# NJU-3DV/Relightable3DGaussian

Hardware: AMD Instinct MI355X
Metric: train iters/s, synthetic lego-like 800x800, 300000 Gaussians (stage-2 hot path) (higher is better)
Workload: dtype f32; 1 GPU; stage-2 train iteration (fused glue kernels + one-launch Adam): shading fwd/bwd (K=64) + rasterize fwd (S=16) + loss + rasterize bwd + Adam; 1 view/rank/step, 300000 Gaussians, 800x800, num_rendered~1755022; parallelism=dp1

## Files before the change

include/r3dg_hip.h:

```cpp
#ifndef R3DG_HIP_H
#define R3DG_HIP_H

#include <stddef.h>
#include <stdint.h>

#ifdef __cplusplus
extern "C" {
#endif

#define R3DG_OK 0
#define R3DG_EINVAL (-1)
#define R3DG_EHIP (-2)
#define R3DG_EALLOC (-3)

typedef void* (*r3dg_alloc_fn)(void* user, size_t bytes);

const char* r3dg_last_error(void);
int r3dg_release_scratch(void);
int r3dg_version(void);

int r3dg_max_features_forward(void);
int r3dg_max_features_backward(void);

size_t r3dg_geometry_state_bytes(int P);
// ... 24 lines not shown
                                 const float* d_rotations, const float* d_cov3D_precomp, const float* d_viewmatrix,
                                 const float* d_projmatrix, const float* d_cam_pos, float tan_fovx, float tan_fovy,
                                 float cx, float cy, int prefiltered, int compute_pseudo_normal, float* d_out_color,
                                 float* d_out_opacity, float* d_out_depth, float* d_out_feature, float* d_out_normal,
                                 float* d_out_surface_xyz, float* d_out_weights, int32_t* d_radii, int debug,
                                 void** ticket);
int r3dg_rasterize_forward_finish(void* ticket, int* num_rendered_out);
int r3dg_rasterize_forward_finish_on(void* ticket, void* ordering_stream, int* num_rendered_out);

int r3dg_bounded_forward_supported(int width, int height);
int r3dg_rasterize_forward_begin_bounded(void* stream, r3dg_alloc_fn geometry_alloc, r3dg_alloc_fn binning_alloc,
                                         r3dg_alloc_fn image_alloc, void* alloc_user, int P, int S, int D, int M,
                                         const float* d_background, int width, int height, const float* d_means3D,
                                         const float* d_shs, const float* d_colors_precomp, const float* d_features,
                                         const float* d_opacities, const float* d_scales, float scale_modifier,
                                         const float* d_rotations, const float* d_cov3D_precomp,
                                         const float* d_viewmatrix, const float* d_projmatrix, const float* d_cam_pos,
                                         float tan_fovx, float tan_fovy, float cx, float cy, int prefiltered,
                                         int compute_pseudo_normal, float* d_out_color, float* d_out_opacity,
                                         float* d_out_depth, float* d_out_feature, float* d_out_normal,
                                         float* d_out_surface_xyz, float* d_out_weights, int32_t* d_radii, int debug,
                                         void* ordering_stream, long long capacity, float* d_overflow_flag,
                                         unsigned int* d_overflow_count, void** ticket);
int r3dg_rasterize_forward_finish_bounded(void* ticket, void* main_stream);

int r3dg_rasterize_backward(void* stream, int P, int S, int D, int M, int R, const float* d_background, int width,
                            int height, const float* d_means3D, const float* d_shs, const float* d_features,
                            const float* d_colors_precomp, const float* d_scales, float scale_modifier,
                            const float* d_rotations, const float* d_cov3D_precomp, const float* d_viewmatrix,
                            const float* d_projmatrix, const float* d_campos, float tan_fovx, float tan_fovy,
                            const int32_t* d_radii, const void* d_geom_buffer, const void* d_binning_buffer,
                            const void* d_img_buffer, const float* d_dL_dpix, const float* d_dL_dpix_o,
                            const float* d_dL_dpix_d, const float* d_dL_dpix_f, float* d_dL_dmean2D,
                            float* d_dL_dconic, float* d_dL_dopacity, float* d_dL_dcolor, float* d_dL_dfeature,
                            float* d_dL_dmean3D, float* d_dL_dcov3D, float* d_dL_dsh, float* d_dL_dscale,
                            float* d_dL_drot, int backward_geometry, int debug);

int r3dg_rasterize_backward_split(void* stream, void* geometry_stream, int P, int S, int D, int M, int R,
                                  const float* d_background, int width, int height, const float* d_means3D,
                                  const float* d_shs, const float* d_features, const float* d_colors_precomp,
                                  const float* d_scales, float scale_modifier, const float* d_rotations,
                                  const float* d_cov3D_precomp, const float* d_viewmatrix, const float* d_projmatrix,
                                  const float* d_campos, float tan_fovx, float tan_fovy, const int32_t* d_radii,
                                  const void* d_geom_buffer, const void* d_binning_buffer, const void* d_img_buffer,
                                  const float* d_dL_dpix, const float* d_dL_dpix_o, const float* d_dL_dpix_d,
                                  const float* d_dL_dpix_f, float* d_dL_dmean2D, float* d_dL_dconic,
// ... 328 lines not shown
```

relightable3dgaussian_amd/csrc/capi_rasterizer.hip:

```cpp
#include "capi_internal.hpp"

#include <mutex>
#include <vector>

namespace r3dg {

GeometryLayout GeometryLayout::make(size_t P)
{
    GeometryLayout L;
    size_t o = 0;
    auto take = [&](size_t bytes) { size_t r = o; o = align_up(o + bytes, 256); return r; };
    L.depths = take(P * 4);
    L.clamped = take(P * 3);
    L.radii = take(P * 4);
    L.means2D = take(P * 8);
    L.cov3D = take(P * 24);
    L.conic_opacity = take(P * 16);
    L.rgb = take(P * 12);
    L.tiles_touched = take(P * 4);
    L.point_offsets = take(P * 4);
    L.block_sums = take(((P + 255) / 256 + 1) * 4);
    L.total = take(8);
    L.splat = take(P * 64);
    L.bytes = o;
// ... 51 lines not shown
        return RasterView{gx, gy, T, N, GeometryLayout::make((size_t)P), ImageLayout::make(N, T)};
    }
};

struct ForwardArgs {
    void* stream;
    r3dg_alloc_fn geometry_alloc, binning_alloc, image_alloc;
    void* user;
    int P, S, D, M;
    const float* background;
    int width, height;
    const float *means3D, *shs, *colors_precomp, *features, *opacities, *scales;
    float scale_modifier;
    const float *rotations, *cov3D_precomp, *viewmatrix, *projmatrix, *cam_pos;
    float tan_fovx, tan_fovy, cx, cy;
    int prefiltered, compute_pseudo_normal;
    float *out_color, *out_opacity, *out_depth, *out_feature, *out_normal, *out_surface_xyz, *out_weights;
    int32_t* radii;
    int debug;
    long long capacity;
    float* overflow_flag;
    unsigned int* overflow_count;
    void* ordering_stream;
};

struct ForwardTicket {
    ForwardArgs a;
    RasterView v;
    float focal_x, focal_y;
    int* radii_p;
    char *gbuf, *ibuf;
    hipEvent_t ready, ordered;
    unsigned long long* host_total;
    char* bbuf;
    bool fused_front;
    uint32_t* point_list;
};

static std::mutex g_ticket_mutex;
static std::vector<ForwardTicket*> g_ticket_pool;

static ForwardTicket* ticket_acquire()
{
    {
        std::lock_guard<std::mutex> lk(g_ticket_mutex);
        if (!g_ticket_pool.empty()) {
// ... 138 lines not shown

    return guarded([&]() -> int {
        hipStream_t stream = (hipStream_t)a.stream;
        const bool debug = a.debug != 0;
        const RasterView v = RasterView::make(a.P, a.width, a.height);
        const GeometryLayout& G = v.G;
        char* gbuf = (char*)a.geometry_alloc(a.user, G.bytes);
        char* ibuf = (char*)a.image_alloc(a.user, v.I.bytes);
        if (!gbuf || !ibuf) { set_error("rasterize_forward: resize callback returned NULL"); return R3DG_EALLOC; }

        ForwardTicket* t = ticket_acquire();
        struct Release { ForwardTicket* t; ~Release() { if (t) ticket_release(t); } } on_error{t};
        t->a = a;
        t->v = v;
        t->focal_y = a.height / (2.0f * a.tan_fovy);
        t->focal_x = a.width / (2.0f * a.tan_fovx);
        t->radii_p = a.radii ? a.radii : (int*)(gbuf + G.radii);
        t->gbuf = gbuf;
        t->ibuf = ibuf;
        t->bbuf = nullptr;
        t->fused_front = false;
        t->point_list = nullptr;
        const hipStream_t order_stream = a.capacity >= 0 && a.ordering_stream ? (hipStream_t)a.ordering_stream : stream;
        stream_wait_stream(order_stream, stream);
        uint32_t* zero_words = nullptr;
        int zero_n = 0;
        if (a.capacity >= 0 && direct_binning_usable((long long)v.T)) {
            BinningLayout B = BinningLayout::make((size_t)a.capacity);
            t->bbuf = (char*)a.binning_alloc(a.user, B.bytes);
            if (!t->bbuf) { set_error("rasterize_forward: binning resize callback returned NULL"); return R3DG_EALLOC; }
            t->fused_front = true;
            zero_words = (uint32_t*)(t->bbuf + B.sort_temp);
            zero_n = (int)v.T;
        }
        unsigned long long* g_total = (unsigned long long*)(gbuf + G.total);
        StageTimer t_pre(order_stream, ST_PREPROCESS);
        launch_preprocess(order_stream, a.P, a.D, a.M, a.means3D, a.scales, a.scale_modifier, a.rotations, a.opacities, a.shs,
                          (uint8_t*)(gbuf + G.clamped), a.cov3D_precomp, a.colors_precomp, a.viewmatrix, a.projmatrix,
                          a.cam_pos, a.width, a.height, a.tan_fovx, a.tan_fovy, t->focal_x, t->focal_y, t->radii_p,
                          (float*)(gbuf + G.means2D), (float*)(gbuf + G.depths), (float*)(gbuf + G.cov3D),
                          (float*)(gbuf + G.rgb), (float*)(gbuf + G.conic_opacity), (float*)(gbuf + G.splat), v.gx, v.gy,
                          (uint32_t*)(gbuf + G.tiles_touched), (uint32_t*)(gbuf + G.block_sums), g_total, !t->fused_front,
                          zero_words, zero_n);
        check_launch(order_stream, debug, "preprocess");
        t_pre.stop();

        if (a.capacity >= 0) {
            const int st_order = enqueue_ordering(t, order_stream, (int)a.capacity);
            if (st_order != R3DG_OK) return st_order;
            R3DG_HIP(hipEventRecord(t->ordered, order_stream));
        } else {
            R3DG_HIP(hipMemcpyAsync(t->host_total, g_total, sizeof(unsigned long long), hipMemcpyDeviceToHost, stream));
            R3DG_HIP(hipEventRecord(t->ready, stream));
        }
        on_error.t = nullptr;
        *ticket_out = t;
        return R3DG_OK;
    });
}

}

using namespace r3dg;

extern "C" {

// ... 34 lines not shown
{
    BinningLayout L = BinningLayout::make((size_t)R);
    o[0] = L.keys_unsorted; o[1] = L.keys; o[2] = L.vals_unsorted; o[3] = L.vals;
    return R3DG_OK;
}

#define R3DG_FORWARD_ARGS                                                                                              \
    stream_, geometry_alloc, binning_alloc, image_alloc, user, P, S, D, M, background, width, height, means3D, shs,    \
        colors_precomp, features, opacities, scales, scale_modifier, rotations, cov3D_precomp, viewmatrix, projmatrix, \
        cam_pos, tan_fovx, tan_fovy, cx, cy, prefiltered, compute_pseudo_normal, out_color, out_opacity, out_depth,    \
        out_feature, out_normal, out_surface_xyz, out_weights, radii, debug_

int r3dg_rasterize_forward_begin(void* stream_, r3dg_alloc_fn geometry_alloc, r3dg_alloc_fn binning_alloc,
                           r3dg_alloc_fn image_alloc, void* user, int P, int S, int D, int M,
                           const float* background, int width, int height, const float* means3D, const float* shs,
                           const float* colors_precomp, const float* features, const float* opacities,
                           const float* scales, float scale_modifier, const float* rotations,
                           const float* cov3D_precomp, const float* viewmatrix, const float* projmatrix,
                           const float* cam_pos, float tan_fovx, float tan_fovy, float cx, float cy, int prefiltered,
                           int compute_pseudo_normal, float* out_color, float* out_opacity, float* out_depth,
                           float* out_feature, float* out_normal, float* out_surface_xyz, float* out_weights,
                           int32_t* radii, int debug_, void** ticket_out)
{
    return forward_begin_impl(ForwardArgs{R3DG_FORWARD_ARGS, -1, nullptr, nullptr, nullptr}, ticket_out);
}

int r3dg_rasterize_forward_begin_bounded(void* stream_, r3dg_alloc_fn geometry_alloc, r3dg_alloc_fn binning_alloc,
                           r3dg_alloc_fn image_alloc, void* user, int P, int S, int D, int M,
                           const float* background, int width, int height, const float* means3D, const float* shs,
                           const float* colors_precomp, const float* features, const float* opacities,
                           const float* scales, float scale_modifier, const float* rotations,
                           const float* cov3D_precomp, const float* viewmatrix, const float* projmatrix,
                           const float* cam_pos, float tan_fovx, float tan_fovy, float cx, float cy, int prefiltered,
                           int compute_pseudo_normal, float* out_color, float* out_opacity, float* out_depth,
                           float* out_feature, float* out_normal, float* out_surface_xyz, float* out_weights,
                           int32_t* radii, int debug_, void* ordering_stream, long long capacity,
                           float* overflow_flag, unsigned int* overflow_count, void** ticket_out)
{
    if (capacity < 0 || capacity > 0x7fffffffll) return invalid("rasterize_forward (bounded): capacity must be in [0, 2^31)");
    return forward_begin_impl(ForwardArgs{R3DG_FORWARD_ARGS, capacity, overflow_flag, overflow_count, ordering_stream},
                              ticket_out);
}
int r3dg_rasterize_forward_finish_bounded(void* ticket_, void* main_stream_)
{
    if (!ticket_) return R3DG_OK;
    ForwardTicket* t = (ForwardTicket*)ticket_;
    if (t->a.capacity < 0) return invalid("rasterize_forward_finish_bounded: not a bounded ticket");
    const int st = guarded([&]() -> int {
        const hipStream_t stream = (hipStream_t)main_stream_;
        R3DG_HIP(hipStreamWaitEvent(stream, t->ordered, 0));
        render_tiles(t, stream);
        return R3DG_OK;
    });
    ticket_release(t);
    return st;
}

int r3dg_rasterize_forward_finish(void* ticket_, int* num_rendered_out)
{
    return r3dg_rasterize_forward_finish_on(ticket_, nullptr, num_rendered_out);
}

int r3dg_rasterize_forward_finish_on(void* ticket_, void* ordering_stream_, int* num_rendered_out)
// ... 16 lines not shown
        if (st_order != R3DG_OK) return st_order;
        stream_wait_stream(main_stream, order_stream);
        render_tiles(t, main_stream);
        if (num_rendered_out) *num_rendered_out = R;
        return R3DG_OK;
    });
    ticket_release(t);
    return st;
}

int r3dg_rasterize_forward(void* stream_, r3dg_alloc_fn geometry_alloc, r3dg_alloc_fn binning_alloc,
                           r3dg_alloc_fn image_alloc, void* user, int P, int S, int D, int M,
                           const float* background, int width, int height, const float* means3D, const float* shs,
                           const float* colors_precomp, const float* features, const float* opacities,
                           const float* scales, float scale_modifier, const float* rotations,
                           const float* cov3D_precomp, const float* viewmatrix, const float* projmatrix,
                           const float* cam_pos, float tan_fovx, float tan_fovy, float cx, float cy, int prefiltered,
                           int compute_pseudo_normal, float* out_color, float* out_opacity, float* out_depth,
                           float* out_feature, float* out_normal, float* out_surface_xyz, float* out_weights,
                           int32_t* radii, int debug_, int* num_rendered_out)
{
    if (num_rendered_out) *num_rendered_out = 0;
    void* ticket = nullptr;
    const int st = forward_begin_impl(ForwardArgs{R3DG_FORWARD_ARGS, -1, nullptr, nullptr, nullptr}, &ticket);
    if (st != R3DG_OK) return st;
    return r3dg_rasterize_forward_finish(ticket, num_rendered_out);
}
#undef R3DG_FORWARD_ARGS

int r3dg_rasterize_backward(void* stream_, int P, int S, int D, int M, int R, const float* background, int width,
                            int height, const float* means3D, const float* shs, const float* features,
                            const float* colors_precomp, const float* scales, float scale_modifier,
                            const float* rotations, const float* cov3D_precomp, const float* viewmatrix,
                            const float* projmatrix, const float* campos, float tan_fovx, float tan_fovy,
                            const int32_t* radii, const void* geom_buffer, const void* binning_buffer,
                            const void* img_buffer, const float* dL_dpix, const float* dL_dpix_o,
                            const float* dL_dpix_d, const float* dL_dpix_f, float* dL_dmean2D, float* dL_dconic,
                            float* dL_dopacity, float* dL_dcolor, float* dL_dfeature, float* dL_dmean3D,
                            float* dL_dcov3D, float* dL_dsh, float* dL_dscale, float* dL_drot,
                            int backward_geometry, int debug_)
{
    return r3dg_rasterize_backward_split(stream_, stream_, P, S, D, M, R, background, width, height, means3D, shs,
                                         features, colors_precomp, scales, scale_modifier, rotations, cov3D_precomp,
                                         viewmatrix, projmatrix, campos, tan_fovx, tan_fovy, radii, geom_buffer,
                                         binning_buffer, img_buffer, dL_dpix, dL_dpix_o, dL_dpix_d, dL_dpix_f, dL_dmean2D,
                                         dL_dconic, dL_dopacity, dL_dcolor, dL_dfeature, dL_dmean3D, dL_dcov3D, dL_dsh,
                                         dL_dscale, dL_drot, backward_geometry, debug_, -1, nullptr);
// ... 138 lines not shown
```

relightable3dgaussian_amd/csrc/launchers.hpp:

```cpp
#pragma once
#include "common.hpp"

namespace r3dg {

constexpr int REFILL_MIN_IDLE = 16;

void release_gradient_records();
void launch_mark_visible(hipStream_t s, int P, const float* means3D, const float* vm, uint8_t* present);
void launch_preprocess(hipStream_t s, int P, int D, int M, const float* means3D, const float* scales, float scale_modifier,
                       const float* rotations, const float* opacities, const float* shs, uint8_t* clamped,
                       const float* cov3D_precomp, const float* colors_precomp, const float* vm, const float* pm,
                       const float* cam_pos, int W, int H, float tan_fovx, float tan_fovy, float focal_x, float focal_y,
                       int* radii, float* means2D, float* depths, float* cov3Ds, float* rgb, float* conic_opacity,
                       float* splat, int gx, int gy, uint32_t* tiles_touched, uint32_t* block_sums,
                       unsigned long long* total, bool scan_now, uint32_t* zero_words, int zero_n);
void launch_duplicate_with_keys(hipStream_t s, int P, const float* means2D, const float* depths,
                                const uint32_t* tiles_touched, const uint32_t* block_offsets, uint32_t* point_offsets,
                                uint64_t* keys, uint32_t* values, const int* radii, int gx, int gy);
void launch_identify_tile_ranges(hipStream_t s, int L, const uint64_t* keys, uint32_t* ranges);
void launch_tile_order(hipStream_t s, int T, const uint32_t* ranges, uint32_t* order, uint32_t small_cap, uint32_t* big_list,
                       uint32_t* big_count);
void launch_render_forward(hipStream_t s, int W, int H, int S, const uint32_t* tile_order, const uint32_t* ranges,
                           const uint32_t* point_list, const float* splat, const float* features, float* final_T,
                           uint32_t* n_contrib, const float* bg, float* out_color, float* out_opacity, float* out_depth,
                           float* out_feature, float* out_weights);
void launch_pseudo_normal(hipStream_t s, int W, int H, const float* vm, float focal_x, float focal_y, float cx, float cy,
                          const float* opacities, const float* depths, float* normals, float* surface_xyz, bool debug);
void launch_render_backward(hipStream_t s, int P, int W, int H, int S, int n_active, const int* active,
                            const uint32_t* tile_order, const uint32_t* ranges, const uint32_t* point_list, const float* bg,
                            const float* splat, const float* features, const float* final_Ts, const uint32_t* n_contrib,
                            const float* dL_dpix, const float* dL_dpix_o, const float* dL_dpix_d, const float* dL_dpix_f,
                            float* dL_dmean2D, float* dL_dconic, float* dL_dopacity, float* dL_dcolor, float* dL_dfeature,
                            int bg_geom);
void launch_render_backward_features(hipStream_t s, int W, int H, int S, int n_active, const int* active,
                                     const uint32_t* tile_order, const uint32_t* ranges, const uint32_t* point_list,
                                     const float* splat, const float* final_Ts, const uint32_t* n_contrib,
                                     const float* dL_dpix_f, float* dL_dfeature);
void launch_preprocess_backward(hipStream_t s, int P, int D, int M, const float* means, const int* radii, const float* shs,
// ... 185 lines not shown
```

relightable3dgaussian_amd/csrc/rasterizer_preprocess.hip:

```cpp
#include <atomic>

#include "launchers.hpp"

namespace r3dg {

struct M3 {
    float c[3][3];
};
__device__ __forceinline__ M3 m3mul(const M3& A, const M3& B)
{
    M3 R;
#pragma unroll
    for (int j = 0; j < 3; j++)
#pragma unroll
        for (int i = 0; i < 3; i++)
            R.c[j][i] = A.c[0][i] * B.c[j][0] + A.c[1][i] * B.c[j][1] + A.c[2][i] * B.c[j][2];
    return R;
}
__device__ __forceinline__ M3 m3t(const M3& A)
{
    M3 R;
#pragma unroll
    for (int j = 0; j < 3; j++)
#pragma unroll
// ... 18 lines not shown
    y0 = min(gy, max(0, f2i_sat((py - max_radius) / R3DG_TILE_Y)));
    x1 = min(gx, max(0, f2i_sat((px + max_radius + R3DG_TILE_X - 1) / R3DG_TILE_X)));
    y1 = min(gy, max(0, f2i_sat((py + max_radius + R3DG_TILE_Y - 1) / R3DG_TILE_Y)));
}

__constant__ float kSH_C0 = 0.28209479177387814f;
__constant__ float kSH_C1 = 0.4886025119029199f;
__constant__ float kSH_C2[5] = {1.0925484305920792f, -1.0925484305920792f, 0.31539156525252005f,
                                -1.0925484305920792f, 0.5462742152960396f};
__constant__ float kSH_C3[7] = {-0.5900435899266435f, 2.890611442640554f, -0.4570457994644658f,
                                0.3731763325901154f, -0.4570457994644658f, 1.445305721320277f,
                                -0.5900435899266435f};

__global__ void mark_visible_kernel(int P, const float* __restrict__ pts, const float* __restrict__ vm,
                                    uint8_t* __restrict__ present)
{
    int idx = blockIdx.x * blockDim.x + threadIdx.x;
    if (idx >= P) return;
    float x = pts[3 * idx], y = pts[3 * idx + 1], z = pts[3 * idx + 2];
    float vz = vm[2] * x + vm[6] * y + vm[10] * z + vm[14];
    present[idx] = vz > 0.2f;
}

template <bool STAGED>
__global__ void __launch_bounds__(256)
preprocess_kernel(int P, int D, int M, const float* __restrict__ means3D, const float* __restrict__ scales,
                  float scale_modifier, const float* __restrict__ rotations, const float* __restrict__ opacities,
                  const float* __restrict__ shs, uint8_t* __restrict__ clamped, const float* __restrict__ cov3D_precomp,
                  const float* __restrict__ colors_precomp, const float* __restrict__ vm,
                  const float* __restrict__ pm, const float* __restrict__ cam_pos, int W, int H, float tan_fovx,
                  float tan_fovy, float focal_x, float focal_y, int* __restrict__ radii,
                  float2* __restrict__ means2D, float* __restrict__ depths, float* __restrict__ cov3Ds,
                  float* __restrict__ rgb, float4* __restrict__ conic_opacity, float4* __restrict__ splat, int gx, int gy,
                  uint32_t* __restrict__ tiles_touched, uint32_t* __restrict__ block_sums,
                  uint32_t* __restrict__ zero_words, int zero_n)
{
    extern __shared__ float s_rows[];
    __shared__ uint8_t s_live[256];
    const int idx = blockIdx.x * 256 + threadIdx.x;
    if (idx < zero_n) zero_words[idx] = 0u;
    uint32_t my_tiles = 0;
    bool shade = false;
    float px = 0.f, py = 0.f, pz = 0.f;
    float4 rec0 = make_float4(0.f, 0.f, 0.f, 0.f), rec1 = rec0;
    if (idx < P) {
        int my_radius_i = 0;
        do {
            px = means3D[3 * idx]; py = means3D[3 * idx + 1]; pz = means3D[3 * idx + 2];
            const float vx = vm[0] * px + vm[4] * py + vm[8] * pz + vm[12];
            const float vy = vm[1] * px + vm[5] * py + vm[9] * pz + vm[13];
            const float vz = vm[2] * px + vm[6] * py + vm[10] * pz + vm[14];
            if (vz <= 0.2f) break;
            const float hx = pm[0] * px + pm[4] * py + pm[8] * pz + pm[12];
            const float hy = pm[1] * px + pm[5] * py + pm[9] * pz + pm[13];
            const float hw = pm[3] * px + pm[7] * py + pm[11] * pz + pm[15];
            const float p_w = 1.0f / (hw + 0.0000001f);
            const float projx = hx * p_w, projy = hy * p_w;

            float c3[6];
            if (cov3D_precomp != nullptr) {
#pragma unroll
                for (int i = 0; i < 6; i++) c3[i] = cov3D_precomp[6 * idx + i];
            } else {
                const float sx = scale_modifier * scales[3 * idx], sy = scale_modifier * scales[3 * idx + 1],
                            sz = scale_modifier * scales[3 * idx + 2];
                const float r = rotations[4 * idx], x = rotations[4 * idx + 1], y = rotations[4 * idx + 2],
                            z = rotations[4 * idx + 3];
                M3 S = {{{sx, 0, 0}, {0, sy, 0}, {0, 0, sz}}};
                M3 R = {{{1.f - 2.f * (y * y + z * z), 2.f * (x * y - r * z), 2.f * (x * z + r * y)},
                         {2.f * (x * y + r * z), 1.f - 2.f * (x * x + z * z), 2.f * (y * z - r * x)},
                         {2.f * (x * z - r * y), 2.f * (y * z + r * x), 1.f - 2.f * (x * x + y * y)}}};
                M3 Mm = m3mul(S, R);
                M3 Sg = m3mul(m3t(Mm), Mm);
                c3[0] = Sg.c[0][0]; c3[1] = Sg.c[0][1]; c3[2] = Sg.c[0][2];
                c3[3] = Sg.c[1][1]; c3[4] = Sg.c[1][2]; c3[5] = Sg.c[2][2];
#pragma unroll
                for (int i = 0; i < 6; i++) cov3Ds[6 * idx + i] = c3[i];
            }

            float tx = vx, ty = vy;
            const float tz = vz;
            const float limx = 1.3f * tan_fovx, limy = 1.3f * tan_fovy;
            const float txtz = tx / tz, tytz = ty / tz;
            tx = fminf(limx, fmaxf(-limx, txtz)) * tz;
            ty = fminf(limy, fmaxf(-limy, tytz)) * tz;
            M3 J = {{{focal_x / tz, 0.0f, -(focal_x * tx) / (tz * tz)},
                     {0.0f, focal_y / tz, -(focal_y * ty) / (tz * tz)},
                     {0, 0, 0}}};
            M3 Wm = {{{vm[0], vm[4], vm[8]}, {vm[1], vm[5], vm[9]}, {vm[2], vm[6], vm[10]}}};
            M3 T = m3mul(Wm, J);
            M3 V = {{{c3[0], c3[1], c3[2]}, {c3[1], c3[3], c3[4]}, {c3[2], c3[4], c3[5]}}};
            M3 cov = m3mul(m3mul(m3t(T), m3t(V)), T);
            const float ca = cov.c[0][0] + 0.3f, cb = cov.c[0][1], cc = cov.c[1][1] + 0.3f;

            const float det = (ca * cc - cb * cb);
            if (det == 0.0f) break;
            const float det_inv = 1.f / det;
            const float mid = 0.5f * (ca + cc);
            const float lambda1 = mid + sqrtf(fmaxf(0.1f, mid * mid - det));
            const float lambda2 = mid - sqrtf(fmaxf(0.1f, mid * mid - det));
            const float my_radius = ceilf(3.f * sqrtf(fmaxf(lambda1, lambda2)));
            const float pixx = ndc_to_pix(projx, W), pixy = ndc_to_pix(projy, H);
            int x0, y0, x1, y1;
            tile_rect(pixx, pixy, f2i_sat(my_radius), gx, gy, x0, y0, x1, y1);
            if ((x1 - x0) * (y1 - y0) == 0) break;

            shade = colors_precomp == nullptr;
            depths[idx] = vz;
            my_radius_i = f2i_sat(my_radius);
            means2D[idx] = make_float2(pixx, pixy);
            const float4 co = make_float4(cc * det_inv, -cb * det_inv, ca * det_inv, opacities[idx]);
            conic_opacity[idx] = co;
            rec0 = make_float4(pixx, pixy, co.x, co.y);
            rec1 = make_float4(co.z, co.w, vz, 0.f);
            my_tiles = (uint32_t)((y1 - y0) * (x1 - x0));
        } while (0);
        radii[idx] = my_radius_i;
        tiles_touched[idx] = my_tiles;
    }
    if (STAGED) {
        s_live[threadIdx.x] = shade;
        __syncthreads();
        stage_rows_in_256(shs, blockIdx.x * 256, P, 3 * M, s_live, s_rows);
        __syncthreads();
    }
    float col[3] = {0.f, 0.f, 0.f};
    if (shade) {
        float dx = px - cam_pos[0], dy = py - cam_pos[1], dz = pz - cam_pos[2];
        const float len = sqrtf(dx * dx + dy * dy + dz * dz);
        dx = dx / len; dy = dy / len; dz = dz / len;
        const float* sh = STAGED ? s_rows + threadIdx.x * staged_row_stride(3 * M) : shs + (size_t)idx * M * 3;
#pragma unroll
        for (int ch = 0; ch < 3; ch++) {
            float result = kSH_C0 * sh[ch];
// ... 507 lines not shown
        total, capacity, nb, (const uint2*)ranges, order, small_cap, big_list, big_count);
}

int tile_binning_max_tiles() { return BIN_MAX_TILES; }

void launch_tile_order(hipStream_t s, int T, const uint32_t* ranges, uint32_t* order, uint32_t small_cap,
                       uint32_t* big_list, uint32_t* big_count)
{
    tile_order_kernel<<<1, 1024, 0, s>>>(T, (const uint2*)ranges, order, small_cap, big_list, big_count);
}

void launch_mark_visible(hipStream_t s, int P, const float* means3D, const float* vm, uint8_t* present)
{
    if (P <= 0) return;
    mark_visible_kernel<<<(P + 255) / 256, 256, 0, s>>>(P, means3D, vm, present);
}

void launch_preprocess(hipStream_t s, int P, int D, int M, const float* means3D, const float* scales,
                       float scale_modifier, const float* rotations, const float* opacities, const float* shs,
                       uint8_t* clamped, const float* cov3D_precomp, const float* colors_precomp, const float* vm,
                       const float* pm, const float* cam_pos, int W, int H, float tan_fovx, float tan_fovy,
                       float focal_x, float focal_y, int* radii, float* means2D, float* depths, float* cov3Ds,
                       float* rgb, float* conic_opacity, float* splat, int gx, int gy, uint32_t* tiles_touched,
                       uint32_t* block_sums, unsigned long long* total, bool scan_now, uint32_t* zero_words, int zero_n)
{
    const int nb = (P + 255) / 256;
    if (zero_n > nb * 256) {
        R3DG_HIP(hipMemsetAsync(zero_words, 0, (size_t)zero_n * 4, s));
        zero_n = 0;
    }
    const bool staged = opt(R3DG_OPT_STAGE_SH_ROWS) && shs != nullptr && colors_precomp == nullptr && M >= 1 && M <= 16;
    if (staged)
        preprocess_kernel<true><<<nb, 256, 256 * ((3 * M) | 1) * sizeof(float), s>>>(
            P, D, M, means3D, scales, scale_modifier, rotations, opacities, shs, clamped, cov3D_precomp, colors_precomp,
            vm, pm, cam_pos, W, H, tan_fovx, tan_fovy, focal_x, focal_y, radii, (float2*)means2D, depths, cov3Ds, rgb,
            (float4*)conic_opacity, (float4*)splat, gx, gy, tiles_touched, block_sums, zero_words, zero_n);
    else
        preprocess_kernel<false><<<nb, 256, 0, s>>>(
            P, D, M, means3D, scales, scale_modifier, rotations, opacities, shs, clamped, cov3D_precomp, colors_precomp,
            vm, pm, cam_pos, W, H, tan_fovx, tan_fovy, focal_x, focal_y, radii, (float2*)means2D, depths, cov3Ds, rgb,
            (float4*)conic_opacity, (float4*)splat, gx, gy, tiles_touched, block_sums, zero_words, zero_n);
    if (scan_now) scan_block_sums_kernel<<<1, 1024, 0, s>>>(nb, block_sums, total);
}

void launch_duplicate_with_keys(hipStream_t s, int P, const float* means2D, const float* depths,
                                const uint32_t* tiles_touched, const uint32_t* block_offsets,
                                uint32_t* point_offsets, uint64_t* keys, uint32_t* values, const int* radii, int gx,
                                int gy)
{
    duplicate_with_keys_kernel<<<(P + 255) / 256, 256, 0, s>>>(P, (const float2*)means2D, depths, tiles_touched,
                                                             block_offsets, point_offsets, keys, values, radii, gx, gy);
}

void launch_identify_tile_ranges(hipStream_t s, int L, const uint64_t* keys, uint32_t* ranges)
{
    if (L <= 0) return;
    identify_tile_ranges_kernel<<<(L + 255) / 256, 256, 0, s>>>(L, keys, (uint2*)ranges);
}

}
```

relightable3dgaussian_amd/csrc/stage2_glue.hip:

```cpp
#include <type_traits>

#include "launchers.hpp"
#include "pseudo_normal.hpp"
#include "r3dg_hip.h"

namespace r3dg {

__device__ __forceinline__ float srgb_pow(float x, float y) { return __builtin_amdgcn_exp2f(y * __builtin_amdgcn_logf(x)); }


__device__ __forceinline__ float sigmoidf_(float x) { return 1.f / (1.f + __expf(-x)); }

__device__ __forceinline__ void normalize3(const float v[3], float eps, float out[3], float& inv)
{
    const float n = sqrtf(v[0] * v[0] + v[1] * v[1] + v[2] * v[2]);
    inv = 1.f / fmaxf(n, eps);
    out[0] = v[0] * inv; out[1] = v[1] * inv; out[2] = v[2] * inv;
}
__device__ __forceinline__ void normalize3_backward(const float v[3], float eps, const float g[3], float out[3])
{
    const float n = sqrtf(v[0] * v[0] + v[1] * v[1] + v[2] * v[2]);
    if (n > eps) {
        const float inv = 1.f / n;
        const float u[3] = {v[0] * inv, v[1] * inv, v[2] * inv};
// ... 20 lines not shown
s2_activate_kernel(int P, const float* __restrict__ xyz, const float* __restrict__ scaling_raw,
                   const float* __restrict__ rotation_raw, const float* __restrict__ opacity_raw,
                   const float* __restrict__ normal_raw, const float* __restrict__ base_raw,
                   const float* __restrict__ rough_raw, const float* __restrict__ campos,
                   float* __restrict__ scales, float* __restrict__ rot, float* __restrict__ opacity,
                   float* __restrict__ normal, float* __restrict__ base_color, float* __restrict__ roughness,
                   float* __restrict__ viewdirs, const float* __restrict__ viewmatrix, float* __restrict__ features,
                   ActivateSide side)
{
    if ((int)blockIdx.x >= side.nb_main) {
        const int nb_side = (int)gridDim.x - side.nb_main;
        for (int k = ((int)blockIdx.x - side.nb_main) * 256 + (int)threadIdx.x; k < side.n_env; k += nb_side * 256) {
            const float r = side.env_raw[k];
            side.env[k] = r > 20.f ? r : log1pf(expf(r));
        }
        for (int k = ((int)blockIdx.x - side.nb_main) * 256 + (int)threadIdx.x; k < side.n_zero; k += nb_side * 256)
            side.zero[k] = 0.f;
        return;
    }
    const int i = blockIdx.x * 256 + threadIdx.x;
    if (i >= P) return;
    const size_t i3 = 3 * (size_t)i, i4 = 4 * (size_t)i;
#pragma unroll
    for (int c = 0; c < 3; c++) scales[i3 + c] = __expf(scaling_raw[i3 + c]);
    {
        const float q[4] = {rotation_raw[i4], rotation_raw[i4 + 1], rotation_raw[i4 + 2], rotation_raw[i4 + 3]};
        const float inv = 1.f / fmaxf(sqrtf(q[0] * q[0] + q[1] * q[1] + q[2] * q[2] + q[3] * q[3]), 1e-12f);
#pragma unroll
        for (int c = 0; c < 4; c++) rot[i4 + c] = q[c] * inv;
    }
    opacity[i] = sigmoidf_(opacity_raw[i]);
    float inv, nrm[3];
    {
        const float v[3] = {normal_raw[i3], normal_raw[i3 + 1], normal_raw[i3 + 2]};
        normalize3(v, 1e-3f, nrm, inv);
        normal[i3] = nrm[0]; normal[i3 + 1] = nrm[1]; normal[i3 + 2] = nrm[2];
    }
    if (base_raw != nullptr) {
        float bc[3];
#pragma unroll
        for (int c = 0; c < 3; c++) base_color[i3 + c] = bc[c] = 0.03f + 0.77f * sigmoidf_(base_raw[i3 + c]);
        const float rg = 0.09f + 0.9f * sigmoidf_(rough_raw[i]);
        roughness[i] = rg;
        const float p[3] = {xyz[i3], xyz[i3 + 1], xyz[i3 + 2]};
        const float d[3] = {campos[0] - p[0], campos[1] - p[1], campos[2] - p[2]};
        float o[3];
        normalize3(d, 1e-12f, o, inv);
        viewdirs[i3] = o[0]; viewdirs[i3 + 1] = o[1]; viewdirs[i3 + 2] = o[2];
        if (features != nullptr) {
            const float depth = p[0] * viewmatrix[2] + p[1] * viewmatrix[6] + p[2] * viewmatrix[10] + viewmatrix[14];
            float* f = features + 16 * (size_t)i;
            *reinterpret_cast<float2*>(f) = make_float2(depth, depth * depth);
            f[5] = nrm[0]; f[6] = nrm[1]; f[7] = nrm[2];
            *reinterpret_cast<float4*>(f + 8) = make_float4(bc[0], bc[1], bc[2], rg);
// ... 1296 lines not shown
```

relightable3dgaussian_amd/fused_step.py:

```python
import collections
import contextlib
import os

import torch
import torch.nn.functional as F

from . import _lib, rasterizer_ops, shading_ops
from .fused_adam import AdamGroup, FusedAdam
from .fused_base import _STREAMS, SUM_SLOTS, FusedStepBase, _in_context, _world_of, grad_slab, learning_rates, shared_stream
from .fused_stage1 import FusedStage1Step
from .grad_comm import BucketComm
from .shading_ops import LEAVE_ROOM, TRAIN_OUTPUTS
from .train_step import FROZEN_GEOMETRY_GROUPS, LAMBDA_DSSIM, STAGE2_WEIGHTS, update_visibility

PARAM_NAMES = ("xyz", "normal", "scaling", "rotation", "opacity", "shs", "base_color", "roughness", "incidents", "env")

_View = collections.namedtuple("_View", "cam bg gt mask H W N vm campos main raw order_stream")


class FusedStage2Step(FusedStepBase):

    _chain_kernel = True
    _opt_order = PARAM_NAMES

# ... 171 lines not shown
            self._skip_cur = flag_cur
            g, active = self._image_loss(v, fw)
            dL_dfeatures, bw, geo_stream, handle_a = self._raster_backward(
                v, fw, g, active, early_adam if split_geometry is None else split_geometry)
            b_early = self._schedule_early(v, handle_a, geo_stream, use_bounded, early_adam, chain_incidents)
            self._shade_backward(v, env_c, taps, packed, dL_dfeatures, bw, geo_stream, b_early, chain_incidents)
            self._remaining_buckets(handle_a)
        return self._end_forward_backward(fw, None if bw is None else bw[0], use_bounded, v.N)

    def _front_end(self, v):
        rotated_for = None
        aux = self._aux_stream()
        if self._chain_deferred is not None:
            self.flush()
        if aux is not None:
            _lib.stream_wait(aux, v.main)
            if not self._rotation_is_current():
                with torch.cuda.stream(aux):
                    self._frs.rotate(self._incidents)
            rotated_for = self._frs
        if self._env_c is None or self._env_c.shape != self.env.shape[1:]:
            self._env_c = torch.empty(tuple(self.env.shape[1:]), dtype=torch.float32, device=self.dev)
        env_c = self._env_c
        self.refresh_activations(v.cam, env_out=env_c, zero=self.sums)
        self._iter += 1
        flag_cur = self._flag_of_iteration()
        use_bounded = self._use_bounded(v.W, v.H)
        if self._early_pending and (aux is None or not (use_bounded and v.order_stream is not None)):
            _lib.stream_wait(v.main, self._adam_stream)
            self._early_pending = False
        if use_bounded:
            bounded = dict(capacity=self._capacity, overflow_flag=flag_cur, overflow_count=self._overflow_count,
                           ordering_stream=v.order_stream)
        else:
            flag_cur.zero_()
            bounded = {}
        cam, empty = v.cam, torch.Tensor([])
        pending = rasterizer_ops.rasterize_gaussians_begin(
            v.bg, self.xyz, self.features, empty, self.a_opacity, self.a_scales, self.a_rot, 1.0, empty, v.vm,
            cam.full_proj_transform, cam.tanfovx, cam.tanfovy, cam.cx, cam.cy, v.H, v.W, self.shs, 3, v.campos, False,
            True, False, want_weights=False,
            defer_pseudo_normal=True, **bounded)
        if self._pending_b is not None:
            self.flush()
        if aux is not None:
            _lib.stream_wait(v.main, aux)
            self._early_pending = False
        return pending, env_c, flag_cur, use_bounded, rotated_for

    def _shade_forward(self, v, env_c, rotated_for):
        L = _lib.lib()
        He, We = env_c.shape[0], env_c.shape[1]
        taps = self.taps(He, We)
        if self._frs is not None:
            rotated = rotated_for is self._frs or (self.dp and self._rotation_is_current())
            self._frs.forward(self.a_base, self.a_rough, self.a_normal, self.a_viewdirs, self._incidents, env_c,
                              self.visibility, self.shade_out, uniform_area=self._uniform_area,
                              leave_room=v.order_stream is not None and not self.dp,
                              listed_stream=self._listed_stream(), rotated=rotated,
                              feature_rows=self.features if self._direct_rows else None)
        else:
            _lib.check(L.r3dg_shade_forward_cached(
                v.raw, self.P, self.K, self.M, self.a_base.data_ptr(), self.a_rough.data_ptr(), self.a_normal.data_ptr(),
                self.a_viewdirs.data_ptr(), self._incidents.data_ptr(), env_c.data_ptr(), He, We, None,
                self.visibility.data_ptr(), self.incident_dirs.data_ptr(),
# ... 250 lines not shown
```

relightable3dgaussian_amd/rasterizer_ops.py:

```python
import ctypes as C

import torch

from . import _lib

NUM_CHANNELS = 3


def _f32c(t):
    if t is None or t.numel() == 0:
        return None
    if t.dtype != torch.float32:
        raise RuntimeError("expected a float32 tensor, got %s" % t.dtype)
    if not t.is_cuda:
        raise RuntimeError("expected a CUDA(HIP) tensor")
    return t.contiguous()


class _Resizer:

    def __init__(self, device):
        self.device = device
        self.buffers = [torch.empty(0, dtype=torch.uint8, device=device) for _ in range(3)]
        self.callbacks = [_lib.ALLOC_FN(self._make(i)) for i in range(3)]
# ... 37 lines not shown
            else:
                with torch.cuda.stream(ordering_stream):
                    st = L.r3dg_rasterize_forward_finish_on(self.ticket, C.c_void_p(ordering_stream.cuda_stream),
                                                            C.byref(rendered))
        self.ticket = None
        geomBuffer, binningBuffer, imgBuffer = self.rs.buffers
        self.rs.callbacks = None
        self.rs = None
        _lib.check(st, "rasterize_gaussians")
        out_color, out_opacity, out_depth, out_feature, out_normal, out_surface_xyz, out_weights, radii = self.outs
        H, W = self.H, self.W
        if imgBuffer.numel() == 0:
            imgBuffer = torch.zeros(int(L.r3dg_image_state_bytes(W, H)), dtype=torch.uint8, device=self.dev)
        off = _offsets(L.r3dg_image_state_offsets, 3, W, H)
        n_contrib = imgBuffer[off[1]:off[1] + 4 * H * W].view(torch.int32).view(H, W)
        return (rendered.value, n_contrib, out_color, out_opacity, out_depth, out_feature, out_normal, out_surface_xyz,
                out_weights, radii, geomBuffer, binningBuffer, imgBuffer)


def rasterize_gaussians_begin(background, means3D, features, colors, opacity, scales, rotations, scale_modifier,
                              cov3D_precomp, viewmatrix, projmatrix, tan_fovx, tan_fovy, cx, cy, image_height,
                              image_width, sh, degree, campos, prefiltered, computer_pseudo_normal, debug,
                              capacity=None, overflow_flag=None, overflow_count=None, ordering_stream=None,
                              want_weights=True, defer_pseudo_normal=False):
    L = _lib.lib()
    if means3D.ndimension() != 2 or means3D.size(1) != 3:
        raise RuntimeError("means3D must have dimensions (num_points, 3)")
    if not means3D.is_cuda:
        raise RuntimeError("means3D must be a CUDA(HIP) tensor")
    P = means3D.size(0)
    S = features.size(1)
    H, W = int(image_height), int(image_width)
    dev = means3D.device
    fopt = dict(dtype=torch.float32, device=dev)

    slab = (torch.zeros if P == 0 else torch.empty)((11 + S, H, W), **fopt)
    out_color, out_opacity, out_depth = slab[0:3], slab[3:4], slab[4:5]
    out_feature, out_normal, out_surface_xyz = slab[5:5 + S], slab[5 + S:8 + S], slab[8 + S:11 + S]
    if defer_pseudo_normal:
        computer_pseudo_normal = False
    elif not computer_pseudo_normal:
        slab[5 + S:].zero_()
    out_weights = torch.zeros((P, 1), **fopt) if want_weights else None
    radii = torch.empty((P,), dtype=torch.int32, device=dev)

    rs = _Resizer(dev)
    ticket = C.c_void_p(None)
    if P != 0:
        M = sh.size(1) if sh.size(0) != 0 else 0
        t = [_f32c(x) for x in (background, means3D, sh, colors, features, opacity, scales, rotations, cov3D_precomp,
                                viewmatrix, projmatrix, campos)]
        bg_, means_, sh_, col_, feat_, op_, sc_, rot_, cov_, vm_, pm_, cam_ = t
        if feat_ is not None and feat_.data_ptr() != features.data_ptr():
            raise RuntimeError("rasterize_gaussians_begin needs contiguous features (their contents are read later)")
        rs.keep = t
        common = (rs.callbacks[0], rs.callbacks[1], rs.callbacks[2], None, P, S, int(degree), M,
                  _lib.ptr(bg_), W, H, _lib.ptr(means_), _lib.ptr(sh_), _lib.ptr(col_), _lib.ptr(feat_), _lib.ptr(op_),
                  _lib.ptr(sc_), float(scale_modifier), _lib.ptr(rot_), _lib.ptr(cov_), _lib.ptr(vm_), _lib.ptr(pm_),
                  _lib.ptr(cam_), float(tan_fovx), float(tan_fovy), float(cx), float(cy), int(bool(prefiltered)),
                  int(bool(computer_pseudo_normal)), out_color.data_ptr(), out_opacity.data_ptr(), out_depth.data_ptr(),
                  _lib.ptr(out_feature), out_normal.data_ptr(), out_surface_xyz.data_ptr(),
                  out_weights.data_ptr() if out_weights is not None else None,
                  radii.data_ptr(), int(bool(debug)))
        with torch.cuda.device(dev):
            if capacity is None:
                st = L.r3dg_rasterize_forward_begin(_lib.current_stream(), *common, C.byref(ticket))
            else:
                if overflow_flag is not None and (overflow_flag.dtype != torch.float32 or not overflow_flag.is_cuda):
                    raise RuntimeError("overflow_flag must be a float32 device tensor")
                if overflow_count is not None and (overflow_count.dtype != torch.int32 or not overflow_count.is_cuda):
                    raise RuntimeError("overflow_count must be an int32 device tensor")
                rs.keep.append((overflow_flag, overflow_count))
                st = L.r3dg_rasterize_forward_begin_bounded(
                    _lib.current_stream(), *common,
                    C.c_void_p(ordering_stream.cuda_stream) if ordering_stream is not None else None, int(capacity),
                    overflow_flag.data_ptr() if overflow_flag is not None else None,
                    overflow_count.data_ptr() if overflow_count is not None else None, C.byref(ticket))
        _lib.check(st, "rasterize_gaussians")
    elif capacity is not None and overflow_flag is not None:
        overflow_flag[:1].zero_()
    return _PendingForward(ticket, rs, (out_color, out_opacity, out_depth, out_feature, out_normal, out_surface_xyz,
                                        out_weights, radii), dev, H, W, capacity=capacity)


def rasterize_gaussians(background, means3D, features, colors, opacity, scales, rotations, scale_modifier,
                        cov3D_precomp, viewmatrix, projmatrix, tan_fovx, tan_fovy, cx, cy, image_height, image_width,
                        sh, degree, campos, prefiltered, computer_pseudo_normal, debug):
    return rasterize_gaussians_begin(background, means3D, features, colors, opacity, scales, rotations, scale_modifier,
                                     cov3D_precomp, viewmatrix, projmatrix, tan_fovx, tan_fovy, cx, cy, image_height,
                                     image_width, sh, degree, campos, prefiltered, computer_pseudo_normal,
                                     debug).finish()


def rasterize_gaussians_backward(background, means3D, features, radii, colors, scales, rotations, scale_modifier,
                                 cov3D_precomp, viewmatrix, projmatrix, tan_fovx, tan_fovy, dL_dout_color,
                                 dL_dout_opacity, dL_dout_depth, dL_dout_feature, sh, degree, campos, geomBuffer, R,
                                 binningBuffer, imageBuffer, backward_geometry, debug, dL_dsh_out=None,
                                 geometry_stream=None, active_features=None, zeroed_accumulators=None):
    L = _lib.lib()
    P = means3D.size(0)
# ... 130 lines not shown
```

Before: 821.3 iters/s.

## Activate raw Gaussian parameters inside preprocess to overlap forward with activation refresh

Adds a raw-parameter bounded forward entry point whose preprocess kernel applies exp, sigmoid and quaternion normalisation itself. The ordering stream now waits on the main stream before the activation refresh is queued, so preprocessing and binning can run concurrently with the glue activation kernel instead of after it. The shared activation helpers keep the fused and glue results consistent. This adds another kernel template variant and a new cross-stream ordering, which carries some risk of synchronisation mistakes.

```diff
diff --git a/include/r3dg_hip.h b/include/r3dg_hip.h
--- a/include/r3dg_hip.h
+++ b/include/r3dg_hip.h
@@ -70,6 +70,19 @@
                                          float* d_out_surface_xyz, float* d_out_weights, int32_t* d_radii, int debug,
                                          void* ordering_stream, long long capacity, float* d_overflow_flag,
                                          unsigned int* d_overflow_count, void** ticket);
+int r3dg_rasterize_forward_begin_bounded_raw(void* stream, r3dg_alloc_fn geometry_alloc, r3dg_alloc_fn binning_alloc,
+                                         r3dg_alloc_fn image_alloc, void* alloc_user, int P, int S, int D, int M,
+                                         const float* d_background, int width, int height, const float* d_means3D,
+                                         const float* d_shs, const float* d_colors_precomp, const float* d_features,
+                                         const float* d_opacities_raw, const float* d_scales_raw, float scale_modifier,
+                                         const float* d_rotations_raw, const float* d_cov3D_precomp,
+                                         const float* d_viewmatrix, const float* d_projmatrix, const float* d_cam_pos,
+                                         float tan_fovx, float tan_fovy, float cx, float cy, int prefiltered,
+                                         int compute_pseudo_normal, float* d_out_color, float* d_out_opacity,
+                                         float* d_out_depth, float* d_out_feature, float* d_out_normal,
+                                         float* d_out_surface_xyz, float* d_out_weights, int32_t* d_radii, int debug,
+                                         void* ordering_stream, long long capacity, float* d_overflow_flag,
+                                         unsigned int* d_overflow_count, int ordering_prequeued, void** ticket);
 int r3dg_rasterize_forward_finish_bounded(void* ticket, void* main_stream);
 
 int r3dg_rasterize_backward(void* stream, int P, int S, int D, int M, int R, const float* d_background, int width,
diff --git a/relightable3dgaussian_amd/csrc/activations.hpp b/relightable3dgaussian_amd/csrc/activations.hpp
--- /dev/null
+++ b/relightable3dgaussian_amd/csrc/activations.hpp
@@ -0,0 +1,23 @@
+#pragma once
+#include <hip/hip_runtime.h>
+
+namespace r3dg {
+
+__device__ __forceinline__ float activate_scale(float raw) { return __expf(raw); }
+
+__device__ __forceinline__ float activate_opacity(float raw)
+{
+#pragma clang fp contract(off)
+    return 1.f / (1.f + __expf(-raw));
+}
+
+__device__ __forceinline__ void activate_rotation(const float q[4], float out[4])
+{
+#pragma clang fp contract(off)
+    const float n2 = ((q[0] * q[0] + q[1] * q[1]) + q[2] * q[2]) + q[3] * q[3];
+    const float inv = 1.f / fmaxf(sqrtf(n2), 1e-12f);
+#pragma unroll
+    for (int c = 0; c < 4; c++) out[c] = q[c] * inv;
+}
+
+}
diff --git a/relightable3dgaussian_amd/csrc/capi_rasterizer.hip b/relightable3dgaussian_amd/csrc/capi_rasterizer.hip
--- a/relightable3dgaussian_amd/csrc/capi_rasterizer.hip
+++ b/relightable3dgaussian_amd/csrc/capi_rasterizer.hip
@@ -97,6 +97,8 @@
     float* overflow_flag;
     unsigned int* overflow_count;
     void* ordering_stream;
+    int raw_params;
+    int ordering_prequeued;
 };
 
 struct ForwardTicket {
@@ -281,7 +283,7 @@
         t->fused_front = false;
         t->point_list = nullptr;
         const hipStream_t order_stream = a.capacity >= 0 && a.ordering_stream ? (hipStream_t)a.ordering_stream : stream;
-        stream_wait_stream(order_stream, stream);
+        if (!a.ordering_prequeued) stream_wait_stream(order_stream, stream);
         uint32_t* zero_words = nullptr;
         int zero_n = 0;
         if (a.capacity >= 0 && direct_binning_usable((long long)v.T)) {
@@ -300,7 +302,7 @@
                           (float*)(gbuf + G.means2D), (float*)(gbuf + G.depths), (float*)(gbuf + G.cov3D),
                           (float*)(gbuf + G.rgb), (float*)(gbuf + G.conic_opacity), (float*)(gbuf + G.splat), v.gx, v.gy,
                           (uint32_t*)(gbuf + G.tiles_touched), (uint32_t*)(gbuf + G.block_sums), g_total, !t->fused_front,
-                          zero_words, zero_n);
+                          zero_words, zero_n, a.raw_params != 0);
         check_launch(order_stream, debug, "preprocess");
         t_pre.stop();
 
@@ -381,7 +383,7 @@
                            float* out_feature, float* out_normal, float* out_surface_xyz, float* out_weights,
                            int32_t* radii, int debug_, void** ticket_out)
 {
-    return forward_begin_impl(ForwardArgs{R3DG_FORWARD_ARGS, -1, nullptr, nullptr, nullptr}, ticket_out);
+    return forward_begin_impl(ForwardArgs{R3DG_FORWARD_ARGS, -1, nullptr, nullptr, nullptr, 0, 0}, ticket_out);
 }
 
 int r3dg_rasterize_forward_begin_bounded(void* stream_, r3dg_alloc_fn geometry_alloc, r3dg_alloc_fn binning_alloc,
@@ -397,7 +399,27 @@
                            float* overflow_flag, unsigned int* overflow_count, void** ticket_out)
 {
     if (capacity < 0 || capacity > 0x7fffffffll) return invalid("rasterize_forward (bounded): capacity must be in [0, 2^31)");
-    return forward_begin_impl(ForwardArgs{R3DG_FORWARD_ARGS, capacity, overflow_flag, overflow_count, ordering_stream},
+    return forward_begin_impl(ForwardArgs{R3DG_FORWARD_ARGS, capacity, overflow_flag, overflow_count, ordering_stream, 0, 0},
+                              ticket_out);
+}
+
+int r3dg_rasterize_forward_begin_bounded_raw(void* stream_, r3dg_alloc_fn geometry_alloc, r3dg_alloc_fn binning_alloc,
+                           r3dg_alloc_fn image_alloc, void* user, int P, int S, int D, int M,
+                           const float* background, int width, int height, const float* means3D, const float* shs,
+                           const float* colors_precomp, const float* features, const float* opacities,
+                           const float* scales, float scale_modifier, const float* rotations,
+                           const float* cov3D_precomp, const float* viewmatrix, const float* projmatrix,
+                           const float* cam_pos, float tan_fovx, float tan_fovy, float cx, float cy, int prefiltered,
+                           int compute_pseudo_normal, float* out_color, float* out_opacity, float* out_depth,
+                           float* out_feature, float* out_normal, float* out_surface_xyz, float* out_weights,
+                           int32_t* radii, int debug_, void* ordering_stream, long long capacity,
+                           float* overflow_flag, unsigned int* overflow_count, int ordering_prequeued, void** ticket_out)
+{
+    if (capacity < 0 || capacity > 0x7fffffffll) return invalid("rasterize_forward (bounded): capacity must be in [0, 2^31)");
+    if (cov3D_precomp != nullptr || opacities == nullptr)
+        return invalid("rasterize_forward (bounded, raw parameters): needs raw opacities, scales and rotations, no precomputed covariance");
+    return forward_begin_impl(ForwardArgs{R3DG_FORWARD_ARGS, capacity, overflow_flag, overflow_count, ordering_stream, 1,
+                                          ordering_prequeued != 0 && ordering_stream != nullptr},
                               ticket_out);
 }
 int r3dg_rasterize_forward_finish_bounded(void* ticket_, void* main_stream_)
@@ -460,7 +482,7 @@
 {
     if (num_rendered_out) *num_rendered_out = 0;
     void* ticket = nullptr;
-    const int st = forward_begin_impl(ForwardArgs{R3DG_FORWARD_ARGS, -1, nullptr, nullptr, nullptr}, &ticket);
+    const int st = forward_begin_impl(ForwardArgs{R3DG_FORWARD_ARGS, -1, nullptr, nullptr, nullptr, 0, 0}, &ticket);
     if (st != R3DG_OK) return st;
     return r3dg_rasterize_forward_finish(ticket, num_rendered_out);
 }
diff --git a/relightable3dgaussian_amd/csrc/launchers.hpp b/relightable3dgaussian_amd/csrc/launchers.hpp
--- a/relightable3dgaussian_amd/csrc/launchers.hpp
+++ b/relightable3dgaussian_amd/csrc/launchers.hpp
@@ -13,7 +13,7 @@
                        const float* cam_pos, int W, int H, float tan_fovx, float tan_fovy, float focal_x, float focal_y,
                        int* radii, float* means2D, float* depths, float* cov3Ds, float* rgb, float* conic_opacity,
                        float* splat, int gx, int gy, uint32_t* tiles_touched, uint32_t* block_sums,
-                       unsigned long long* total, bool scan_now, uint32_t* zero_words, int zero_n);
+                       unsigned long long* total, bool scan_now, uint32_t* zero_words, int zero_n, bool raw_params);
 void launch_duplicate_with_keys(hipStream_t s, int P, const float* means2D, const float* depths,
                                 const uint32_t* tiles_touched, const uint32_t* block_offsets, uint32_t* point_offsets,
                                 uint64_t* keys, uint32_t* values, const int* radii, int gx, int gy);
diff --git a/relightable3dgaussian_amd/csrc/rasterizer_preprocess.hip b/relightable3dgaussian_amd/csrc/rasterizer_preprocess.hip
--- a/relightable3dgaussian_amd/csrc/rasterizer_preprocess.hip
+++ b/relightable3dgaussian_amd/csrc/rasterizer_preprocess.hip
@@ -1,5 +1,6 @@
 #include <atomic>
 
+#include "activations.hpp"
 #include "launchers.hpp"
 
 namespace r3dg {
@@ -64,7 +65,7 @@
     present[idx] = vz > 0.2f;
 }
 
-template <bool STAGED>
+template <bool STAGED, bool RAW>
 __global__ void __launch_bounds__(256)
 preprocess_kernel(int P, int D, int M, const float* __restrict__ means3D, const float* __restrict__ scales,
                   float scale_modifier, const float* __restrict__ rotations, const float* __restrict__ opacities,
@@ -104,10 +105,16 @@
 #pragma unroll
                 for (int i = 0; i < 6; i++) c3[i] = cov3D_precomp[6 * idx + i];
             } else {
-                const float sx = scale_modifier * scales[3 * idx], sy = scale_modifier * scales[3 * idx + 1],
-                            sz = scale_modifier * scales[3 * idx + 2];
-                const float r = rotations[4 * idx], x = rotations[4 * idx + 1], y = rotations[4 * idx + 2],
-                            z = rotations[4 * idx + 3];
+                float s3[3] = {scales[3 * idx], scales[3 * idx + 1], scales[3 * idx + 2]};
+                float q[4] = {rotations[4 * idx], rotations[4 * idx + 1], rotations[4 * idx + 2], rotations[4 * idx + 3]};
+                if (RAW) {
+                    const float q_raw[4] = {q[0], q[1], q[2], q[3]};
+                    activate_rotation(q_raw, q);
+#pragma unroll
+                    for (int c = 0; c < 3; c++) s3[c] = activate_scale(s3[c]);
+                }
+                const float sx = scale_modifier * s3[0], sy = scale_modifier * s3[1], sz = scale_modifier * s3[2];
+                const float r = q[0], x = q[1], y = q[2], z = q[3];
                 M3 S = {{{sx, 0, 0}, {0, sy, 0}, {0, 0, sz}}};
                 M3 R = {{{1.f - 2.f * (y * y + z * z), 2.f * (x * y - r * z), 2.f * (x * z + r * y)},
                          {2.f * (x * y + r * z), 1.f - 2.f * (x * x + z * z), 2.f * (y * z - r * x)},
@@ -151,7 +158,8 @@
             depths[idx] = vz;
             my_radius_i = f2i_sat(my_radius);
             means2D[idx] = make_float2(pixx, pixy);
-            const float4 co = make_float4(cc * det_inv, -cb * det_inv, ca * det_inv, opacities[idx]);
+            const float4 co = make_float4(cc * det_inv, -cb * det_inv, ca * det_inv,
+                                          RAW ? activate_opacity(opacities[idx]) : opacities[idx]);
             conic_opacity[idx] = co;
             rec0 = make_float4(pixx, pixy, co.x, co.y);
             rec1 = make_float4(co.z, co.w, vz, 0.f);
@@ -705,7 +713,8 @@
                        const float* pm, const float* cam_pos, int W, int H, float tan_fovx, float tan_fovy,
                        float focal_x, float focal_y, int* radii, float* means2D, float* depths, float* cov3Ds,
                        float* rgb, float* conic_opacity, float* splat, int gx, int gy, uint32_t* tiles_touched,
-                       uint32_t* block_sums, unsigned long long* total, bool scan_now, uint32_t* zero_words, int zero_n)
+                       uint32_t* block_sums, unsigned long long* total, bool scan_now, uint32_t* zero_words, int zero_n,
+                       bool raw_params)
 {
     const int nb = (P + 255) / 256;
     if (zero_n > nb * 256) {
@@ -713,16 +722,17 @@
         zero_n = 0;
     }
     const bool staged = opt(R3DG_OPT_STAGE_SH_ROWS) && shs != nullptr && colors_precomp == nullptr && M >= 1 && M <= 16;
-    if (staged)
-        preprocess_kernel<true><<<nb, 256, 256 * ((3 * M) | 1) * sizeof(float), s>>>(
+    auto launch = [&](auto kernel, size_t lds) {
+        kernel<<<nb, 256, lds, s>>>(
             P, D, M, means3D, scales, scale_modifier, rotations, opacities, shs, clamped, cov3D_precomp, colors_precomp,
             vm, pm, cam_pos, W, H, tan_fovx, tan_fovy, focal_x, focal_y, radii, (float2*)means2D, depths, cov3Ds, rgb,
             (float4*)conic_opacity, (float4*)splat, gx, gy, tiles_touched, block_sums, zero_words, zero_n);
+    };
+    const size_t lds = staged ? 256 * ((3 * M) | 1) * sizeof(float) : 0;
+    if (staged)
+        raw_params ? launch(preprocess_kernel<true, true>, lds) : launch(preprocess_kernel<true, false>, lds);
     else
-        preprocess_kernel<false><<<nb, 256, 0, s>>>(
-            P, D, M, means3D, scales, scale_modifier, rotations, opacities, shs, clamped, cov3D_precomp, colors_precomp,
-            vm, pm, cam_pos, W, H, tan_fovx, tan_fovy, focal_x, focal_y, radii, (float2*)means2D, depths, cov3Ds, rgb,
-            (float4*)conic_opacity, (float4*)splat, gx, gy, tiles_touched, block_sums, zero_words, zero_n);
+        raw_params ? launch(preprocess_kernel<false, true>, lds) : launch(preprocess_kernel<false, false>, lds);
     if (scan_now) scan_block_sums_kernel<<<1, 1024, 0, s>>>(nb, block_sums, total);
 }
 
diff --git a/relightable3dgaussian_amd/csrc/stage2_glue.hip b/relightable3dgaussian_amd/csrc/stage2_glue.hip
--- a/relightable3dgaussian_amd/csrc/stage2_glue.hip
+++ b/relightable3dgaussian_amd/csrc/stage2_glue.hip
@@ -1,5 +1,6 @@
 #include <type_traits>
 
+#include "activations.hpp"
 #include "launchers.hpp"
 #include "pseudo_normal.hpp"
 #include "r3dg_hip.h"
@@ -66,14 +67,15 @@
     if (i >= P) return;
     const size_t i3 = 3 * (size_t)i, i4 = 4 * (size_t)i;
 #pragma unroll
-    for (int c = 0; c < 3; c++) scales[i3 + c] = __expf(scaling_raw[i3 + c]);
+    for (int c = 0; c < 3; c++) scales[i3 + c] = activate_scale(scaling_raw[i3 + c]);
     {
         const float q[4] = {rotation_raw[i4], rotation_raw[i4 + 1], rotation_raw[i4 + 2], rotation_raw[i4 + 3]};
-        const float inv = 1.f / fmaxf(sqrtf(q[0] * q[0] + q[1] * q[1] + q[2] * q[2] + q[3] * q[3]), 1e-12f);
-#pragma unroll
-        for (int c = 0; c < 4; c++) rot[i4 + c] = q[c] * inv;
-    }
-    opacity[i] = sigmoidf_(opacity_raw[i]);
+        float u[4];
+        activate_rotation(q, u);
+#pragma unroll
+        for (int c = 0; c < 4; c++) rot[i4 + c] = u[c];
+    }
+    opacity[i] = activate_opacity(opacity_raw[i]);
     float inv, nrm[3];
     {
         const float v[3] = {normal_raw[i3], normal_raw[i3 + 1], normal_raw[i3 + 2]};
diff --git a/relightable3dgaussian_amd/fused_step.py b/relightable3dgaussian_amd/fused_step.py
--- a/relightable3dgaussian_amd/fused_step.py
+++ b/relightable3dgaussian_amd/fused_step.py
@@ -217,10 +217,14 @@
         if self._env_c is None or self._env_c.shape != self.env.shape[1:]:
             self._env_c = torch.empty(tuple(self.env.shape[1:]), dtype=torch.float32, device=self.dev)
         env_c = self._env_c
-        self.refresh_activations(v.cam, env_out=env_c, zero=self.sums)
         self._iter += 1
         flag_cur = self._flag_of_iteration()
         use_bounded = self._use_bounded(v.W, v.H)
+        raw_front = (use_bounded and v.order_stream is not None and v.order_stream is not v.main
+                     and not (self._early_pending and aux is None))
+        if raw_front:
+            _lib.stream_wait(v.order_stream, v.main)
+        self.refresh_activations(v.cam, env_out=env_c, zero=self.sums)
         if self._early_pending and (aux is None or not (use_bounded and v.order_stream is not None)):
             _lib.stream_wait(v.main, self._adam_stream)
             self._early_pending = False
@@ -231,11 +235,12 @@
             flag_cur.zero_()
             bounded = {}
         cam, empty = v.cam, torch.Tensor([])
+        geo = (self.opacity, self.scaling, self.rotation) if raw_front else (self.a_opacity, self.a_scales, self.a_rot)
         pending = rasterizer_ops.rasterize_gaussians_begin(
-            v.bg, self.xyz, self.features, empty, self.a_opacity, self.a_scales, self.a_rot, 1.0, empty, v.vm,
+            v.bg, self.xyz, self.features, empty, *geo, 1.0, empty, v.vm,
             cam.full_proj_transform, cam.tanfovx, cam.tanfovy, cam.cx, cam.cy, v.H, v.W, self.shs, 3, v.campos, False,
             True, False, want_weights=False,
-            defer_pseudo_normal=True, **bounded)
+            defer_pseudo_normal=True, raw_params=raw_front, ordering_prequeued=raw_front, **bounded)
         if self._pending_b is not None:
             self.flush()
         if aux is not None:
diff --git a/relightable3dgaussian_amd/rasterizer_ops.py b/relightable3dgaussian_amd/rasterizer_ops.py
--- a/relightable3dgaussian_amd/rasterizer_ops.py
+++ b/relightable3dgaussian_amd/rasterizer_ops.py
@@ -83,7 +83,8 @@
                               cov3D_precomp, viewmatrix, projmatrix, tan_fovx, tan_fovy, cx, cy, image_height,
                               image_width, sh, degree, campos, prefiltered, computer_pseudo_normal, debug,
                               capacity=None, overflow_flag=None, overflow_count=None, ordering_stream=None,
-                              want_weights=True, defer_pseudo_normal=False):
+                              want_weights=True, defer_pseudo_normal=False, raw_params=False,
+                              ordering_prequeued=False):
     L = _lib.lib()
     if means3D.ndimension() != 2 or means3D.size(1) != 3:
         raise RuntimeError("means3D must have dimensions (num_points, 3)")
@@ -124,6 +125,8 @@
                   out_weights.data_ptr() if out_weights is not None else None,
                   radii.data_ptr(), int(bool(debug)))
         with torch.cuda.device(dev):
+            if raw_params and capacity is None:
+                raise RuntimeError("rasterize_gaussians_begin: raw_params needs the bounded forward (capacity)")
             if capacity is None:
                 st = L.r3dg_rasterize_forward_begin(_lib.current_stream(), *common, C.byref(ticket))
             else:
@@ -132,11 +135,14 @@
                 if overflow_count is not None and (overflow_count.dtype != torch.int32 or not overflow_count.is_cuda):
                     raise RuntimeError("overflow_count must be an int32 device tensor")
                 rs.keep.append((overflow_flag, overflow_count))
-                st = L.r3dg_rasterize_forward_begin_bounded(
-                    _lib.current_stream(), *common,
-                    C.c_void_p(ordering_stream.cuda_stream) if ordering_stream is not None else None, int(capacity),
-                    overflow_flag.data_ptr() if overflow_flag is not None else None,
-                    overflow_count.data_ptr() if overflow_count is not None else None, C.byref(ticket))
+                tail = (C.c_void_p(ordering_stream.cuda_stream) if ordering_stream is not None else None, int(capacity),
+                        overflow_flag.data_ptr() if overflow_flag is not None else None,
+                        overflow_count.data_ptr() if overflow_count is not None else None)
+                if raw_params:
+                    st = L.r3dg_rasterize_forward_begin_bounded_raw(_lib.current_stream(), *common, *tail,
+                                                                    int(bool(ordering_prequeued)), C.byref(ticket))
+                else:
+                    st = L.r3dg_rasterize_forward_begin_bounded(_lib.current_stream(), *common, *tail, C.byref(ticket))
         _lib.check(st, "rasterize_gaussians")
     elif capacity is not None and overflow_flag is not None:
         overflow_flag[:1].zero_()
```

Result: slower. 810.7 iters/s (-1.3%).
